# asmirnou/watsor

Hardware: AMD Instinct MI355X
Metric: detected frames/sec (whole node) + p50 per-frame latency, SSD-MobileNet 300x300 (higher is better)
Workload: dtype f16; 1 GPU; 1 synthetic 640x480 RGB stream per GPU, batch=8 frames, SSD-MobileNet-v2 300x300 (seeded random-init weights), frames resident in HBM, rows copied back to host; batch=8, frame=640x480, parallelism=replica-per-gpu x1, batches_in_flight=4, graph_nodes_per_batch=31

## Files before the change

### watsor_amd/csrc/k_conv.hip

```cpp
#include "wz_common.h"

__global__ __launch_bounds__(256) void wz_k_stem(const half_t* __restrict__ in, const float* __restrict__ w,
                                                 const float* __restrict__ bias, half_t* __restrict__ out,
                                                 int total, int hin, int win, int hout, int wout, int pad_t,
                                                 int pad_l) {
    __shared__ float sw[27 * 32 + 32];
    for (int i = threadIdx.x; i < 27 * 32; i += 256) sw[i] = w[i];
    if (threadIdx.x < 32) sw[27 * 32 + threadIdx.x] = bias[threadIdx.x];
    __syncthreads();
    const int tid = blockIdx.x * 256 + threadIdx.x;
    if (tid >= total) return;
    const int cg = tid & 3, pix = tid >> 2;
    const int ox = pix % wout;
    const int t2 = pix / wout;
    const int oy = t2 % hout, b = t2 / hout;
    float acc[8];
#pragma unroll
    for (int j = 0; j < 8; ++j) acc[j] = sw[27 * 32 + cg * 8 + j];
#pragma unroll
    for (int ky = 0; ky < 3; ++ky) {
        const int iy = oy * 2 - pad_t + ky;
        if (iy < 0 || iy >= hin) continue;
#pragma unroll
        for (int kx = 0; kx < 3; ++kx) {
            const int ix = ox * 2 - pad_l + kx;
            if (ix < 0 || ix >= win) continue;
            const half4_t p = *reinterpret_cast<const half4_t*>(in + ((size_t)(b * hin + iy) * win + ix) * 4);
#pragma unroll
            for (int c = 0; c < 3; ++c) {
                const float x = (float)p[c];
                const float* wr = sw + ((ky * 3 + kx) * 3 + c) * 32 + cg * 8;
#pragma unroll
                for (int j = 0; j < 8; ++j) acc[j] = fmaf(x, wr[j], acc[j]);
            }
        }
    }
    half8_t o;
#pragma unroll
    for (int j = 0; j < 8; ++j) o[j] = (half_t)fminf(fmaxf(acc[j], 0.0f), 6.0f);
    *reinterpret_cast<half8_t*>(out + (size_t)pix * 32 + cg * 8) = o;
}

void wz_launch_stem(const half_t* in, const float* w, const float* bias, half_t* out, int n, int hin, int win,
                    int hout, int wout, int pad_t, int pad_l, hipStream_t s) {
    const int total = n * hout * wout * 4;
    WZ_LAUNCH(wz_k_stem, dim3((total + 255) / 256), dim3(256), 0, s, in, w, bias, out, total, hin, win,
                       hout, wout, pad_t, pad_l);
}

__global__ __launch_bounds__(256) void wz_k_dw(const half_t* __restrict__ in, const half_t* __restrict__ w,
                                               const float* __restrict__ bias, half_t* __restrict__ out,
                                               int total, int hin, int win, int c, int hout, int wout, int stride,
                                               int pad_t, int pad_l, int act) {
    const int tid = blockIdx.x * 256 + threadIdx.x;
    if (tid >= total) return;
    const int c8 = c >> 3;
    const int cg = tid % c8, pix = tid / c8;
    const int ox = pix % wout;
    const int t2 = pix / wout;
    const int oy = t2 % hout, b = t2 / hout;
    float acc[8];
    {
        const float4_t b0 = *reinterpret_cast<const float4_t*>(bias + cg * 8);
        const float4_t b1 = *reinterpret_cast<const float4_t*>(bias + cg * 8 + 4);
#pragma unroll
        for (int j = 0; j < 4; ++j) { acc[j] = b0[j]; acc[4 + j] = b1[j]; }
    }
#pragma unroll
    for (int ky = 0; ky < 3; ++ky) {
        const int iy = oy * stride - pad_t + ky;
        if (iy < 0 || iy >= hin) continue;
#pragma unroll
        for (int kx = 0; kx < 3; ++kx) {
            const int ix = ox * stride - pad_l + kx;
            if (ix < 0 || ix >= win) continue;
            const half8_t x = *reinterpret_cast<const half8_t*>(in + ((size_t)(b * hin + iy) * win + ix) * c + cg * 8);
            const half8_t k = *reinterpret_cast<const half8_t*>(w + (size_t)(ky * 3 + kx) * c + cg * 8);
#pragma unroll
            for (int j = 0; j < 8; ++j) acc[j] = fmaf((float)x[j], (float)k[j], acc[j]);
        }
    }
    half8_t o;
#pragma unroll
    for (int j = 0; j < 8; ++j) {
        float v = acc[j];
        if (act == WZ_ACT_RELU6) v = fminf(fmaxf(v, 0.0f), 6.0f);
        o[j] = (half_t)v;
    }
    *reinterpret_cast<half8_t*>(out + (size_t)pix * c + cg * 8) = o;
}

void wz_launch_dw(const half_t* in, const half_t* w, const float* bias, half_t* out, int n, int hin, int win,
                  int c, int hout, int wout, int stride, int pad_t, int pad_l, int act, hipStream_t s) {
    const int total = n * hout * wout * (c >> 3);
    WZ_LAUNCH(wz_k_dw, dim3((total + 255) / 256), dim3(256), 0, s, in, w, bias, out, total, hin, win, c,
                       hout, wout, stride, pad_t, pad_l, act);
}


__device__ __forceinline__ void wz_epilogue4(const WzConvArgs& a, int m, int n4, float4_t v) {
    if (m >= a.M || n4 >= a.cout) return;
    const float4_t bv = *reinterpret_cast<const float4_t*>(a.bias + n4);
#pragma unroll
    for (int r = 0; r < 4; ++r) {
        float x = v[r] + bv[r];
        if (a.act == WZ_ACT_RELU6) x = fminf(fmaxf(x, 0.0f), 6.0f);
        v[r] = x;
    }
    if (a.out_mode == WZ_OUT_ACT) {
        const size_t o = (size_t)m * a.cout + n4;
        if (a.res) {
            const half4_t rv = *reinterpret_cast<const half4_t*>(a.res + o);
#pragma unroll
            for (int r = 0; r < 4; ++r) v[r] += (float)rv[r];
        }
        half4_t h = {(half_t)v[0], (half_t)v[1], (half_t)v[2], (half_t)v[3]};
        const size_t os = a.out_cstride ? (size_t)m * a.out_cstride + a.out_coff + n4 : o;
        *reinterpret_cast<half4_t*>(reinterpret_cast<half_t*>(a.out) + os) = h;
    } else {
        const int hw = a.hout * a.wout;
        const int b = m / hw, pix = m - b * hw;
        float* o;
        int cols, n0;
        if (a.out_mode == WZ_OUT_HEAD && n4 >= a.n_box) {
            cols = a.cout - a.n_box;
            n0 = n4 - a.n_box;
            o = a.out2 + (size_t)b * a.out2_batch_stride + a.out2_off;
        } else {
            cols = (a.out_mode == WZ_OUT_HEAD) ? a.n_box : a.cout;
            n0 = n4;
            o = reinterpret_cast<float*>(a.out) + (size_t)b * a.out_batch_stride + a.out_off;
        }
        o += (size_t)pix * cols + n0;
#pragma unroll
        for (int r = 0; r < 4; ++r)
            if (n0 + r < cols) o[r] = v[r];
    }
}

__device__ __forceinline__ void wz_decode_anchor(const float4_t e, const float4_t an, const WzPostConsts& k,
                                                 float* __restrict__ box_out, uint8_t* __restrict__ valid_out) {
#pragma clang fp contract(off)
    const float ty = e[0] / k.scale_y, tx = e[1] / k.scale_x, th = e[2] / k.scale_h, tw = e[3] / k.scale_w;
    const float w = expf(tw) * an[3];
    const float h = expf(th) * an[2];
    const float yc = ty * an[2] + an[0];
    const float xc = tx * an[3] + an[1];
    const float hh = h / 2.0f, hw = w / 2.0f;
    float ymin = yc - hh, xmin = xc - hw, ymax = yc + hh, xmax = xc + hw;
    if (k.clip_after) {
        *reinterpret_cast<float4_t*>(box_out) = (float4_t){ymin, xmin, ymax, xmax};
        *valid_out = 1;
        return;
    }
    ymin = fminf(fmaxf(ymin, 0.0f), 1.0f);
    xmin = fminf(fmaxf(xmin, 0.0f), 1.0f);
    ymax = fminf(fmaxf(ymax, 0.0f), 1.0f);
    xmax = fminf(fmaxf(xmax, 0.0f), 1.0f);
    const float area = (ymax - ymin) * (xmax - xmin);
    *reinterpret_cast<float4_t*>(box_out) = (float4_t){ymin, xmin, ymax, xmax};
    *valid_out = area > 0.0f ? 1 : 0;
}

__device__ __forceinline__ void wz_head_finish(const WzConvArgs& a, int m, int n4, float4_t v, bool list, bool decode,
                                               const float* __restrict__ hint_logit, uint32_t* __restrict__ cbits,
                                               int cbits_words, const WzPostConsts& pc, const float* __restrict__ anchors,
                                               float* __restrict__ boxes, uint8_t* __restrict__ valid) {
    wz_epilogue4(a, m, n4, v);
    if (m >= a.M) return;
    const int n_box = a.out_mode == WZ_OUT_HEAD ? a.n_box : (a.out_mode == WZ_OUT_BOX ? a.cout : 0);
    if (list && n4 >= n_box && n4 < a.cout && a.out_mode != WZ_OUT_BOX && a.out_mode != WZ_OUT_ACT) {
        const int hw = a.hout * a.wout;
        const int b = m / hw, pix = m - b * hw;
        const int cols = a.cout - n_box, n0 = n4 - n_box;
        const long long off = a.out_mode == WZ_OUT_HEAD ? a.out2_off : a.out_off;
        const float lf = hint_logit[b];
        const float4_t bv = *reinterpret_cast<const float4_t*>(a.bias + n4);
#pragma unroll
        for (int r = 0; r < 4; ++r) {
            const float x = v[r] + bv[r];
            if (n0 + r < cols && x >= lf) {
                const long long j = off + (long long)pix * cols + n0 + r;
                atomicOr(&cbits[(size_t)b * cbits_words + (size_t)(j >> 5)], 1u << (j & 31));
            }
        }
    }
    if (decode && n4 < n_box) {
        const float4_t bv = *reinterpret_cast<const float4_t*>(a.bias + n4);
        float4_t enc;
#pragma unroll
        for (int r = 0; r < 4; ++r) enc[r] = v[r] + bv[r];
        const int hw = a.hout * a.wout;
        const int b = m / hw, pix = m - b * hw;
        const int anchor = (int)(a.out_off >> 2) + pix * (n_box >> 2) + (n4 >> 2);
        const size_t i = (size_t)b * pc.num_anchors + anchor;
        wz_decode_anchor(enc, *reinterpret_cast<const float4_t*>(anchors + (size_t)anchor * 4), pc, boxes + i * 4, valid + i);
    }
}


template <int MT, int NT, int U>
struct ConvFrags {
    half8_t xa[U][MT];
    half8_t wf[U][NT];
};

template <int KS, int MT, int NT, int U>
__device__ __forceinline__ void wz_conv_load(const WzConvArgs& a, ConvFrags<MT, NT, U>& f, int& ql, const int q1, int& t,
                                             int& c, const int (&iy0)[MT], const int (&ix0)[MT],
                                             const int (&boff)[MT], const bool (&mv)[MT],
                                             const half_t* wlane, const int nt0, const int cg8) {
    constexpr int taps = KS * KS;
    const half8_t zero = {0, 0, 0, 0, 0, 0, 0, 0};
#pragma unroll
    for (int u = 0; u < U; ++u) {
        const bool live = ql < q1;
        const int ky = (KS == 1) ? 0 : t / KS, kx = (KS == 1) ? 0 : t - ky * KS;
        const bool cin_ok = (c * 32 + cg8) < a.cin;
#pragma unroll
        for (int mt = 0; mt < MT; ++mt) {
            const int iy = iy0[mt] + ky, ix = ix0[mt] + kx;
            const bool ok = live && cin_ok && mv[mt] && iy >= 0 && iy < a.hin && ix >= 0 && ix < a.win;
            f.xa[u][mt] = ok ? *reinterpret_cast<const half8_t*>(
                                   a.in + ((size_t)(boff[mt] + iy) * a.win + ix) * a.cin + c * 32 + cg8)
                             : zero;
        }
#pragma unroll
        for (int nt = 0; nt < NT; ++nt)
            f.wf[u][nt] = live ? *reinterpret_cast<const half8_t*>(
                                     wlane + ((size_t)((nt0 + nt) * taps + t) * a.kc + c) * 512)
                               : zero;
        ++ql;
        if (++c == a.kc) {
            c = 0;
            ++t;
        }
    }
}

template <int MT, int NT, int U>
__device__ __forceinline__ void wz_conv_mfma(const ConvFrags<MT, NT, U>& f, float4_t (&acc)[MT][NT]) {
#pragma unroll
    for (int u = 0; u < U; ++u)
#pragma unroll
        for (int mt = 0; mt < MT; ++mt)
#pragma unroll
            for (int nt = 0; nt < NT; ++nt)
                acc[mt][nt] = __builtin_amdgcn_mfma_f32_16x16x32_f16(f.wf[u][nt], f.xa[u][mt], acc[mt][nt], 0, 0, 0);
}

template <int KS, int MT, int NT, int U>
__device__ __forceinline__ void wz_conv_body(const WzConvArgs& a, int bx, int by, int bz) {
    const int lane = threadIdx.x & 63;
    const int wave = threadIdx.x >> 6;
    const int r16 = lane & 15, g = lane >> 4;
    const int m_base = (bx * 4 + wave) * (MT * 16);
    const int nt0 = by * NT;
    if (m_base >= a.M) return;

    const int hw = a.hout * a.wout;
    int iy0[MT], ix0[MT], boff[MT];
    bool mv[MT];
#pragma unroll
    for (int mt = 0; mt < MT; ++mt) {
        const int m = m_base + mt * 16 + r16;
        mv[mt] = m < a.M;
        const int mm = mv[mt] ? m : 0;
        const int b = mm / hw, rem = mm - b * hw;
        const int oy = rem / a.wout, ox = rem - oy * a.wout;
        iy0[mt] = oy * a.stride - a.pad_t;
        ix0[mt] = ox * a.stride - a.pad_l;
        boff[mt] = b * a.hin;
    }

    float4_t acc[MT][NT];
#pragma unroll
    for (int mt = 0; mt < MT; ++mt)
#pragma unroll
        for (int nt = 0; nt < NT; ++nt) acc[mt][nt] = (float4_t){0.f, 0.f, 0.f, 0.f};

    const int per = (a.kchunks + a.splitk - 1) / a.splitk;
    const int q0 = bz * per;
    const int q1 = min(q0 + per, a.kchunks);
    const half_t* wlane = a.w + (size_t)lane * 8;
    const int cg8 = g * 8;

    int ql = q0, t = (KS == 1) ? 0 : q0 / a.kc, c = (KS == 1) ? q0 : q0 - t * a.kc;
    ConvFrags<MT, NT, U> fa, fb;
    wz_conv_load<KS, MT, NT, U>(a, fa, ql, q1, t, c, iy0, ix0, boff, mv, wlane, nt0, cg8);
    for (int q = q0; q < q1;) {
        wz_conv_load<KS, MT, NT, U>(a, fb, ql, q1, t, c, iy0, ix0, boff, mv, wlane, nt0, cg8);
// ... 356 lines not shown
```

### watsor_amd/csrc/wz_common.h

```cpp
#pragma once
#include <hip/hip_runtime.h>
#include <hip/hip_fp16.h>
#include <stdint.h>
#include <stdlib.h>

#include "../../include/watsor_hip.h"
#include "wz_program.h"

typedef _Float16 half_t;
typedef __attribute__((ext_vector_type(8))) _Float16 half8_t;
typedef __attribute__((ext_vector_type(4))) _Float16 half4_t;
typedef __attribute__((ext_vector_type(4))) float float4_t;
#ifdef __HIPCC__
__device__ __forceinline__ half4_t wz_relu6_pack(const float4_t d, const float4_t bv, bool keep) {
    typedef __attribute__((ext_vector_type(2))) unsigned int wz_uint2_t;
    half4_t o;
#pragma unroll
    for (int r = 0; r < 4; ++r) o[r] = (half_t)fminf(fmaxf(d[r] + bv[r], 0.0f), 6.0f);
    wz_uint2_t p = __builtin_bit_cast(wz_uint2_t, o);
    p[0] = keep ? p[0] : 0u;
    p[1] = keep ? p[1] : 0u;
    return __builtin_bit_cast(half4_t, p);
}
#endif

struct WzFrameDesc {
    const uint8_t* rgb;
    int32_t w, h;
    float scale_x, scale_y;
    int32_t cam;
    int32_t fmt;
};
static_assert(sizeof(WzFrameDesc) == 32, "WzFrameDesc is 32 bytes (WzDescPack, the lanes' descriptor blocks)");

struct WzConvArgs {
    const half_t* in;
    const half_t* w;
    const float* bias;
    const half_t* res;
    void* out;
    int32_t M;
    int32_t hin, win, cin;
    int32_t hout, wout, cout, n_pad;
    int32_t ksize, stride, pad_t, pad_l, kc;
    int32_t act, out_mode;
    int32_t splitk;
    int32_t kchunks;
    int64_t out_batch_stride;
    int64_t out_off;
    float* out2;
    int64_t out2_batch_stride, out2_off;
    int32_t n_box;
    const half_t* zeros;
    int32_t grid_m, grid_n;
    float* ws;
    unsigned long long* dbg;
    int32_t nt_base;
    int32_t nt_live, nt_group;
    int32_t frag_ws;
    int32_t out_coff, out_cstride;
};


struct WzPostConsts {
    int32_t num_anchors, num_classes;
    int32_t max_total, max_per_class;
    float score_thr, iou_thr;
    float scale_y, scale_x, scale_h, scale_w;
    int32_t clip_after;
    int32_t _pad;
};

struct WzMbArgs {
    const half_t* in;
    const half_t* we;
    const float* be;
    const half_t* wd;
    const float* bd;
    const half_t* wp;
    const float* bp;
    const half_t* res;
    half_t* out;
    int32_t hin, win, hout, wout;
    int32_t cin0, kc0, nmid_pad;
    int32_t cmid, cmid_pad, kc;
    int32_t cout, n_pad;
    int32_t stride, pad_t, pad_l;
    int32_t stem, sin_h, sin_w, spad_t, spad_l;
    float* ws;
    uint64_t ws_bytes;
    int32_t M;
    unsigned long long* dbg;
    int32_t th, tw, tiles_y, tiles_x, nsplit, cpg, stage, ebufs, nb;
    const half_t* we_lo;
    const half_t* wp_lo;
    int32_t hp, hp_out;
    half_t* out2;
    int32_t has_out2;
    int32_t qenc;
    unsigned long long* dbg2;
    int32_t lone;
};

struct WzDwsepArgs {
    const half_t* in;
    const half_t* wd;
    const float* bd;
    const half_t* wp;
    const float* bp;
    half_t* out;
    int32_t M;
    int32_t hin, win, hout, wout;
    int32_t cin, kc, cout, n_pad;
    int32_t stride, pad_t, pad_l;
    unsigned long long* dbg;
};

struct WzCamFilter {
    int32_t enabled, width, height, n_zones;
    const int32_t* sat;
    double conf_thr[WZ_NUM_LABELS];
    double area_thr[WZ_NUM_LABELS];
    uint8_t allow[WZ_NUM_LABELS][WZ_MAX_ZONES * 4];
};
#define WZ_MAX_ZONES_PER_CAM (WZ_MAX_ZONES * 4)


extern thread_local int wz_launch_repeat;
static inline const char* wz_dev_getenv(const char* name) {
#ifdef WZ_DEV_BUILD
    return getenv(name);
#else
    (void)name;
    return nullptr;
#endif
}
static inline int wz_dev_env_int(const char* name, int dflt) {
    const char* e = wz_dev_getenv(name);
    return (e && e[0] && atoi(e) >= 0) ? atoi(e) : dflt;
}

bool wz_latency_schedule();

#ifndef WZ_LANE_STAMPS
#define WZ_LANE_STAMPS 0
#endif
#define WZ_STAMP_SLOTS 128
#define WZ_STAMP_WORDS 384
#define WZ_STAMP_ENTRY 16
#define WZ_STAMP_EXIT 80
#define WZ_STAMP_PRE_BYTES (WZ_STAMP_WORDS * 8)
struct WzLaunchNote { const void* func; unsigned grid[3], block[3]; unsigned lds; };
#if WZ_LANE_STAMPS
void wz_note_launch(const void* func, dim3 grid, dim3 block, size_t lds);
#define WZ_LAUNCH(kern, grid, block, lds, s, ...) do { wz_note_launch(reinterpret_cast<const void*>(kern), grid, block, lds); \
        for (int _wz_r = 0; _wz_r < wz_launch_repeat; ++_wz_r) hipLaunchKernelGGL(kern, grid, block, lds, s, __VA_ARGS__); } while (0)
#ifdef __HIPCC__
struct WzLaneStamp {
    unsigned long long* p;
    __device__ __forceinline__ explicit WzLaneStamp(unsigned long long* q) : p(q) {
        if (p && threadIdx.x == 0 && threadIdx.y == 0 && threadIdx.z == 0) {
            const unsigned id = blockIdx.x + gridDim.x * (blockIdx.y + gridDim.y * blockIdx.z);
            if (id < 64u) p[WZ_STAMP_ENTRY + id] = (unsigned long long)wall_clock64();
        }
    }
    __device__ __forceinline__ ~WzLaneStamp() {
        if (p && threadIdx.x == 0 && threadIdx.y == 0 && threadIdx.z == 0) {
            const unsigned id = blockIdx.x + gridDim.x * (blockIdx.y + gridDim.y * blockIdx.z);
            p[WZ_STAMP_EXIT + (id & 255u)] = (unsigned long long)wall_clock64();
        }
    }
};
#define WZ_LANE_STAMP(ptr) WzLaneStamp _wz_lane_stamp(const_cast<unsigned long long*>(ptr))
#endif
#else
#define WZ_LAUNCH(...) do { for (int _wz_r = 0; _wz_r < wz_launch_repeat; ++_wz_r) hipLaunchKernelGGL(__VA_ARGS__); } while (0)
#define WZ_LANE_STAMP(ptr) do { } while (0)
#endif
#define WZ_DESC_PACK 16
struct WzDescPack { WzFrameDesc d[WZ_DESC_PACK]; };
void wz_launch_preprocess(const WzFrameDesc* d_frames, int n, int size, half_t* out, hipStream_t s, bool hp = false,
                          WzFrameDesc* keep = nullptr, bool half_pixel = false, const WzFrameDesc* by_value = nullptr, int rows_lds = 0);
size_t wz_preprocess_rows_lds(int max_w);
size_t wz_preprocess_rows_need(int w, int fmt);
int wz_preprocess_flags(bool half_pixel, int rows_lds);
int wz_preprocess_rows_threads();
const void* wz_preprocess_func(bool hp, bool rows = false);
void wz_launch_stem(const half_t* in, const float* w, const float* bias, half_t* out, int n, int hin, int win,
                    int hout, int wout, int pad_t, int pad_l, hipStream_t s);
void wz_launch_dw(const half_t* in, const half_t* w, const float* bias, half_t* out, int n, int hin, int win,
                  int c, int hout, int wout, int stride, int pad_t, int pad_l, int act, hipStream_t s);
void wz_launch_conv(const WzConvArgs& a, hipStream_t s);
void wz_launch_splitk_reduce(const WzConvArgs& a, const float* ws, hipStream_t s);
#define WZ_REDUCE_GROUP_MAX 8
struct WzReduceGroup {
    int32_t n;
    int32_t first[WZ_REDUCE_GROUP_MAX + 1];
    WzConvArgs a[WZ_REDUCE_GROUP_MAX];
    const float* ws[WZ_REDUCE_GROUP_MAX];
    int32_t decode;
    int32_t list, cbits_words;
    unsigned long long* stamp;
    const float* hint_logit;
    uint32_t* cbits;
    WzPostConsts pc;
    const float* anchors;
    float* boxes;
    uint8_t* valid;
};
void wz_reduce_group_add(WzReduceGroup& g, const WzConvArgs& a, const float* ws);
#define WZ_CONV_GROUP_MAX 6
struct WzConvGroup {
    int32_t n;
    int32_t first[WZ_CONV_GROUP_MAX + 1];
    int32_t gx[WZ_CONV_GROUP_MAX], gy[WZ_CONV_GROUP_MAX];
    WzConvArgs a[WZ_CONV_GROUP_MAX];
    unsigned long long* stamp;
};
bool wz_conv_ws_applies(const WzConvArgs& a);
void wz_launch_conv_ws(const WzConvArgs& a, hipStream_t s);
bool wz_conv_groupable(const WzConvArgs& a);
void wz_conv_group_add(WzConvGroup& g, const WzConvArgs& a);
void wz_launch_conv_group(const WzConvGroup& g, hipStream_t s);
bool wz_conv_rs_groupable(const WzConvArgs& a);
int wz_conv_rs_group_add(WzConvGroup& g, const WzConvArgs& a);
void wz_launch_conv_rs_group(const WzConvGroup& g, hipStream_t s);
bool wz_conv_wide_applies(const WzConvArgs& a);
#define WZ_WIDE_TILES 12
void wz_conv_wide_shape(const WzConvArgs& a, int* tiles, int* steps);
int wz_choose_wide_T(const int* tiles, const int* steps, const long long* tile_bytes, int n, int cus);
int wz_conv_wide_group_add(WzConvGroup& g, const WzConvArgs& a);
void wz_launch_conv_wide_group(const WzConvGroup& g, hipStream_t s);
void wz_launch_splitk_reduce_group(const WzReduceGroup& g, hipStream_t s);
int wz_choose_splitk(int M, int n_pad, int kchunks);
bool wz_conv_use_lds(const WzConvArgs& a);
int wz_choose_splitk_lds(int M, int n_pad, int kchunks);
int wz_lds_nw(int M, int n_pad, int kchunks);
bool wz_conv_f32_use_rs(const WzConvArgs& a);
int wz_choose_splitk_rs_f32(int M, int n_pad, int kchunks);
bool wz_conv_ws_f32_applies(const WzConvArgs& a);
void wz_launch_conv_ws_f32(const WzConvArgs& a, hipStream_t s);
bool wz_extras_pair_applies(const WzConvArgs& a, const WzConvArgs& b);
void wz_launch_extras_pair(const WzConvArgs& a, const WzConvArgs& b, int n, hipStream_t s);
void wz_launch_stem_f32(const half_t* in, const float* w, const float* bias, float* out, int n, int hin, int win,
                        int hout, int wout, int pad_t, int pad_l, hipStream_t s, bool pair = false);
void wz_launch_dw_f32(const float* in, const float* w, const float* bias, float* out, int n, int hin, int win, int c,
                      int hout, int wout, int stride, int pad_t, int pad_l, int act, hipStream_t s);
void wz_launch_conv_f32(const WzConvArgs& a, hipStream_t s, bool reduce = true);
void wz_launch_stem7(const half_t* in, const half_t* w, const float* bias, half_t* out, int n, int hin, int win, int hout, int wout,
                     int pad_t, int pad_l, int cstride, int coff, hipStream_t s);
void wz_launch_stem7_f32(const half_t* in, const float* w, const float* bias, float* out, int n, int hin, int win, int hout, int wout,
                         int pad_t, int pad_l, int cstride, int coff, bool pair, hipStream_t s);
void wz_launch_pool3(const half_t* in, half_t* out, int n, int hin, int win, int c, int hout, int wout, int stride, int pad_t, int pad_l,
                     bool is_max, int cstride, int coff, hipStream_t s);
void wz_launch_pool3_f32(const float* in, float* out, int n, int hin, int win, int c, int hout, int wout, int stride, int pad_t, int pad_l,
                         bool is_max, int cstride, int coff, hipStream_t s);
int wz_launch_mbconv(const WzMbArgs& a, int n, hipStream_t s, bool prepare);
int wz_launch_mbconv_wave(const WzMbArgs& a, int n, hipStream_t s, bool prepare);
int wz_launch_mbconv_cs(const WzMbArgs& a, int n, hipStream_t s, bool prepare);
int wz_launch_mbconv_hp(const WzMbArgs& a, int n, hipStream_t s, bool prepare);
int wz_mbconv_hp2_applies(const WzMbArgs& a, int n);
int wz_launch_mbconv_hp2(const WzMbArgs& a, int n, hipStream_t s, bool prepare, int phase);
int wz_launch_dwsep(const WzDwsepArgs& a, hipStream_t s, bool prepare);

#define WZ_HIST_BINS 1024
#define WZ_CAND_CAP 4096
#define WZ_NMS_KEEP_MAX 128
#define WZ_CAND_TARGET 192
struct WzPostBuffers {
    uint32_t* hint;
    float* hint_logit;
    uint32_t* cbits;
    const float* box_enc;
    const float* logits;
    const float* anchors;
    float* boxes;
    uint8_t* valid;
    float* det_boxes;
    float* det_scores;
    int32_t* det_classes;
    int32_t* det_num;
    unsigned long long* dbg;
    unsigned long long* stamps;
    unsigned long long* stamps_pre;
    unsigned long long* stamps_host;
    int32_t stamps_n, _stamps_pad;
};
void wz_launch_decode(const WzPostBuffers& b, const WzPostConsts& c, int n, hipStream_t s);
void wz_launch_nms(const WzPostBuffers& b, const WzPostConsts& c, int n, hipStream_t s, const WzFrameDesc* d_frames = nullptr,
                   const WzCamFilter* d_cams = nullptr, wz_detection_t* rows = nullptr, uint8_t* pass = nullptr,
                   bool listed = false, uint32_t* status = nullptr);
void wz_launch_rows(const WzPostBuffers& b, const WzFrameDesc* d_frames, const WzCamFilter* d_cams, int n,
                    int max_total, wz_detection_t* rows, uint8_t* pass, hipStream_t s);
int wz_set_error(int code, const char* fmt, ...);
void wz_post_init();
void wz_launch_filter_rows(const WzCamFilter* d_cams, int cam, wz_detection_t* rows, uint8_t* pass, hipStream_t s);
void wz_launch_sat(const uint8_t* fill, int32_t* sat, int width, int height, int n_zones, hipStream_t s);

struct WzCropPlane {
    const uint8_t* src;
    uint8_t* dst;
    int32_t src_pitch, row_bytes, rows, _pad;
};
#define WZ_CROP_PACK 48
struct WzCropPack { WzCropPlane p[WZ_CROP_PACK]; };
struct WzMergeFrame { int32_t first, n_tiles, cam, _pad; };
struct WzMergeCand {
    int32_t label, x_min, y_min, x_max, y_max, _pad;
    double confidence;
};
void wz_launch_crop_tiles(const WzCropPlane* planes, int n, hipStream_t s);
void wz_launch_merge_tiles(const WzMergeFrame* frames, const int32_t* origins, const wz_detection_t* tile_rows, WzMergeCand* cands, int n,
                           int max_tiles, double iou_thr, double ios_thr, wz_detection_t* rows, uint8_t* pass, hipStream_t s);

#define WZ_GATE_GRAY 0
#define WZ_GATE_YUYV 1
#define WZ_GATE_UYVY 2
#define WZ_GATE_RGB 3
#define WZ_GATE_BGR 4
#define WZ_GATE_LOW10 5
struct WzGateTile {
    const uint8_t* src;
    const uint16_t* ref;
    uint16_t* now;
    int32_t pitch, row_bytes, tw, th, cols, crows, mode, thr;
};
struct WzGateCommit {
    uint16_t* ref;
    const uint16_t* now;
    wz_detection_t* cache;
    int32_t cells, fresh;
};
void wz_launch_tile_activity(const WzGateTile* tiles, int n, int max_crows, int max_cols, int32_t* counters, int32_t* activity, hipStream_t s);
void wz_launch_gate_commit(const WzGateCommit* tiles, int n, const wz_detection_t* batch_rows, wz_detection_t* out, hipStream_t s);
```

### watsor_amd/csrc/wz_engine.hip

```cpp
#include <math.h>
#include <stdarg.h>
#include <stdio.h>
#include <stdlib.h>
#include <string.h>

#include <algorithm>
#include <atomic>
#include <chrono>

#include "wz_engine.h"

static const char kHwQueuesVar[] = "GPU_MAX_HW_QUEUES";
static const int kHwQueuesNeeded = 8;
static int wz_env_hw_queues() {
    const char* v = getenv(kHwQueuesVar);
    if (!v || !v[0]) return 0;
    char* end = nullptr;
    const long n = strtol(v, &end, 10);
    while (*end == ' ' || *end == '\t') ++end;
    return (*end || n < 1 || n > 1 << 20) ? 0 : (int)n;
}
#ifndef WZ_KEEP_HOST_HW_QUEUES
__attribute__((constructor)) static void wz_runtime_defaults() {
    if (wz_env_hw_queues() < kHwQueuesNeeded) setenv(kHwQueuesVar, "8", 1);
// ... 208 lines not shown
            if (e->d_mbdbg) e->mb_groups[i] = groups;
            if (t) t->mark();
            if (groups > 1) {
                WzConvArgs r;
                memset(&r, 0, sizeof(r));
                r.bias = a.bp; r.res = a.res; r.out = a.out;
                r.M = a.M; r.hout = op.hout; r.wout = op.wout; r.cout = op.cout; r.n_pad = op.n_pad;
                r.act = WZ_ACT_NONE; r.out_mode = WZ_OUT_ACT; r.splitk = groups;
                WZ_STAMP_ARG(r);
                wz_launch_splitk_reduce(r, L.d_ws, s);
            }
        } else {
            if (!f32 && op.out_mode == WZ_OUT_ACT && op.ksize == 1 && op.dst_c == 0 && i + 1 < e->hdr.n_ops) {
                const WzOpDesc& nx = e->ops[i + 1];
                bool only = nx.kind == WZ_OP_CONV && nx.src == op.dst && nx.out_mode == WZ_OUT_ACT && op.res < 0 && nx.res < 0 &&
                            nx.dst_c == 0;
                for (uint32_t j = 0; only && j < e->hdr.n_ops; ++j)
                    if (j != i + 1 && (e->ops[j].src == op.dst || e->ops[j].res == op.dst)) only = false;
                if (only) {
                    auto conv_args = [&](const WzOpDesc& o) {
                        WzConvArgs c;
                        memset(&c, 0, sizeof(c));
                        c.in = L.tptr[o.src];
                        c.w = (const half_t*)(wbase + o.w_off);
                        c.bias = (const float*)(wbase + o.b_off);
                        c.out = L.tptr[o.dst];
                        c.M = n * o.hout * o.wout;
                        c.hin = o.hin; c.win = o.win; c.cin = o.cin;
                        c.hout = o.hout; c.wout = o.wout; c.cout = o.cout; c.n_pad = o.n_pad;
                        c.ksize = o.ksize; c.stride = o.stride; c.pad_t = o.pad_t; c.pad_l = o.pad_l; c.kc = o.kc;
                        c.act = o.act; c.out_mode = o.out_mode;
                        c.kchunks = o.ksize * o.ksize * o.kc;
                        c.splitk = 1;
                        return c;
                    };
                    WzConvArgs pa = conv_args(op);
                    const WzConvArgs pb = conv_args(nx);
                    if (wz_extras_pair_applies(pa, pb)) {
                        WZ_STAMP_ARG(pa);
                        wz_launch_extras_pair(pa, pb, n, s);
                        if (t) { t->mark(); t->mark(); t->mark(); t->mark(); }
                        ++i;
                        continue;
                    }
                }
            }
            WzConvArgs a;
            memset(&a, 0, sizeof(a));
            a.in = L.tptr[op.src];
            a.w = (const half_t*)(wbase + op.w_off);
            a.bias = (const float*)(wbase + op.b_off);
            a.res = op.res >= 0 ? L.tptr[op.res] : nullptr;
            a.M = n * op.hout * op.wout;
            a.hin = op.hin; a.win = op.win; a.cin = op.cin;
            a.hout = op.hout; a.wout = op.wout; a.cout = op.cout; a.n_pad = op.n_pad;
            a.ksize = op.ksize; a.stride = op.stride; a.pad_t = op.pad_t; a.pad_l = op.pad_l; a.kc = op.kc;
            a.act = op.act; a.out_mode = op.out_mode;
            a.kchunks = op.ksize * op.ksize * op.kc;
            if (op.out_mode == WZ_OUT_ACT && op.dst_c != 0) {
                a.out_cstride = op.dst_c;
                a.out_coff = op.dst_coff;
            }
            void* final_out;
            if (op.out_mode == WZ_OUT_ACT) {
                final_out = L.tptr[op.dst];
            } else if (op.out_mode == WZ_OUT_BOX) {
                final_out = L.d_box_enc;
                a.out_batch_stride = (int64_t)e->hdr.num_anchors * 4;
                a.out_off = (int64_t)op.anchor_off * 4;
            } else if (op.out_mode == WZ_OUT_CLS) {
                final_out = L.d_logits;
                a.out_batch_stride = (int64_t)e->hdr.num_anchors * e->hdr.num_classes;
                a.out_off = (int64_t)op.anchor_off * e->hdr.num_classes;
            } else {
                final_out = L.d_box_enc;
                a.out_batch_stride = (int64_t)e->hdr.num_anchors * 4;
                a.out_off = (int64_t)op.anchor_off * 4;
                a.out2 = L.d_logits;
                a.out2_batch_stride = (int64_t)e->hdr.num_anchors * e->hdr.num_classes;
                a.out2_off = (int64_t)op.anchor_off * e->hdr.num_classes;
                a.n_box = op.n_box;
            }
            a.zeros = e->d_zeros;
            a.dbg = e->d_mbdbg ? e->d_mbdbg + (size_t)i * 16 : nullptr;
            const bool makes_boxes = op.out_mode == WZ_OUT_HEAD || op.out_mode == WZ_OUT_BOX;
            if (makes_boxes) ++box_ops;
            if (op.out_mode != WZ_OUT_ACT) ++head_ops;
            if (f32) {
                int sk = !e->use_splitk ? 1 : wz_conv_f32_use_rs(a) ? wz_choose_splitk_rs_f32(a.M, a.n_pad, a.kchunks) : wz_choose_splitk(a.M, a.n_pad, a.kchunks / 2);
                const size_t slab32 = (((size_t)sk * a.M * a.n_pad * 4) + 255) & ~(size_t)255;
                if (sk > 1 && e->defer_heads && op.out_mode != WZ_OUT_ACT && heads.n < WZ_REDUCE_GROUP_MAX &&
                    slab32 + (e->ws_bytes >> 1) <= ws_top) {
                    ws_top -= slab32;
                    float* const park = reinterpret_cast<float*>(reinterpret_cast<unsigned char*>(L.d_ws) + ws_top);
                    a.splitk = sk;
                    a.ws = park;
                    a.out = final_out;
                    wz_launch_conv_f32(a, s, false);
                    if (t) { t->mark(); t->mark(); }
                    wz_reduce_group_add(heads, a, park);
                    if (makes_boxes) ++box_ops_grouped;
                    continue;
                }
                if (wz_conv_ws_f32_applies(a)) {
                    a.splitk = 1;
                    a.out = final_out;
                    wz_launch_conv_ws_f32(a, s);
                    if (t) { t->mark(); t->mark(); }
                    continue;
                }
                while (sk > 1 && (size_t)sk * a.M * a.n_pad * 4 > ws_top) --sk;
                a.splitk = sk;
                a.ws = L.d_ws;
                a.out = final_out;
                wz_launch_conv_f32(a, s);
                if (t) { t->mark(); t->mark(); }
                continue;
            }
            int sk = 1;
            if (e->use_splitk)
                sk = wz_conv_use_lds(a) ? wz_choose_splitk_lds(a.M, a.n_pad, a.kchunks) : wz_choose_splitk(a.M, a.n_pad, a.kchunks);
            bool to_wide = wide_T > 0 && wide.n < WZ_CONV_GROUP_MAX && wz_conv_wide_applies(a) && a.M >= e->wide_min_m;
            const size_t m16 = ((size_t)a.M + 15) & ~(size_t)15;
            if (to_wide) {
                const int wsk = ((a.kchunks >> 1) + wide_T - 1) / wide_T;
                if (heads.n < WZ_REDUCE_GROUP_MAX && ((((size_t)wsk * m16 * a.n_pad * 4) + 255) & ~(size_t)255) + (e->ws_bytes >> 1) <= ws_top)
                    sk = wsk;
                else
                    to_wide = false;
            }
            a.frag_ws = to_wide ? 1 : 0;
            const size_t slab = (((size_t)sk * (to_wide ? m16 : (size_t)a.M) * a.n_pad * 4) + 255) & ~(size_t)255;
            if ((sk > 1 || to_wide) && e->defer_heads && op.out_mode != WZ_OUT_ACT && heads.n < WZ_REDUCE_GROUP_MAX &&
                slab + (e->ws_bytes >> 1) <= ws_top) {
                ws_top -= slab;
                float* const park = reinterpret_cast<float*>(reinterpret_cast<unsigned char*>(L.d_ws) + ws_top);
                a.splitk = sk;
                a.out = park;
                if (to_wide) {
                    wz_conv_wide_group_add(wide, a);
                } else if (small.n < WZ_CONV_GROUP_MAX && wz_conv_groupable(a)) {
                    wz_conv_group_add(small, a);
                } else if (!(wz_conv_rs_groupable(a) && wz_conv_rs_group_add(big, a))) {
                    WZ_STAMP_ARG(a);
                    wz_launch_conv(a, s);
                }
                if (t) { t->mark(); t->mark(); }
                a.out = final_out;
                wz_reduce_group_add(heads, a, park);
                if (makes_boxes) ++box_ops_grouped;
                continue;
            }
            a.frag_ws = 0;
            if ((sk > 1 || a.M < 128) && wz_conv_ws_applies(a)) {
                a.splitk = 1;
                a.out = final_out;
                WZ_STAMP_ARG(a);
                wz_launch_conv_ws(a, s);
                if (t) { t->mark(); t->mark(); }
                continue;
            }
            while (sk > 1 && (size_t)sk * a.M * a.n_pad * 4 > ws_top) --sk;
            a.splitk = sk;
            if (sk > 1) {
                a.out = L.d_ws;
                WZ_STAMP_ARG(a);
                wz_launch_conv(a, s);
                if (t) t->mark();
                a.out = final_out;
                WZ_STAMP_ARG(a);
                wz_launch_splitk_reduce(a, L.d_ws, s);
            } else {
                a.out = final_out;
                WZ_STAMP_ARG(a);
                wz_launch_conv(a, s);
                if (t) t->mark();
            }
        }
        if (t) t->mark();
    }
    L.decode_fused = heads.n > 0 && box_ops > 0 && box_ops == box_ops_grouped && e->fuse_decode;
    L.cands_listed = with_post && L.decode_fused && head_ops == heads.n;
    wide.stamp = big.stamp = small.stamp = heads.stamp = nullptr;
    if (wide.n > 0) { WZ_STAMP_GROUP(wide); wz_launch_conv_wide_group(wide, s); }
    if (big.n > 0) { WZ_STAMP_GROUP(big); wz_launch_conv_rs_group(big, s); }
    if (t) t->mark();
    if (small.n > 0) { WZ_STAMP_GROUP(small); wz_launch_conv_group(small, s); }
    if (t) t->mark();
    if (L.decode_fused) {
        heads.decode = 1;
        heads.pc = e->pc;
        heads.anchors = L.post.anchors;
        heads.boxes = L.post.boxes;
        heads.valid = L.post.valid;
    }
    heads.list = L.cands_listed ? 1 : 0;
    if (L.cands_listed) {
        heads.hint_logit = L.post.hint_logit;
        heads.cbits = L.post.cbits;
        heads.cbits_words = (e->pc.num_anchors * e->pc.num_classes + 31) >> 5;
    }
    if (heads.n > 0) { WZ_STAMP_GROUP(heads); wz_launch_splitk_reduce_group(heads, s); }
    if (t) t->mark();
}

static void enqueue_post(wz_engine* e, Lane& L, bool rows, int n, StageTimer* t, bool decode_done = false, bool listed = false) {
    hipStream_t s = L.stream;
    if (!decode_done) wz_launch_decode(L.post, e->pc, n, s);
    if (t) t->mark();
#if WZ_LANE_STAMPS
    L.post.stamps_n = rows && L.m_stamps ? L.stamp_next : 0;
    L.post.stamps_host = rows && L.post.stamps_n ? L.m_stamps : nullptr;
#endif
    if (rows)
        wz_launch_nms(L.post, e->pc, n, s, L.d_desc, e->d_cams, L.m_rows, L.m_pass, listed, L.m_status);
    else
        wz_launch_nms(L.post, e->pc, n, s, nullptr, nullptr, nullptr, nullptr, listed);
    if (t) t->mark();
    if (rows && t) t->mark();
}

static void enqueue_batch(wz_engine* e, Lane& L, int n, StageTimer* t, int inner = 1) {
    hipStream_t s = L.stream;
    if (t) t->mark();
    const bool by_value = e->desc_by_value && n <= WZ_DESC_PACK;
    const bool zero_copy = !by_value && e->desc_zero_copy && L.h_desc_dev;
    if (!by_value && !zero_copy) (void)hipMemcpyAsync(L.d_desc, L.h_desc, sizeof(WzFrameDesc) * n, hipMemcpyHostToDevice, s);
    if (t) t->mark();
    wz_launch_repeat = inner;
    L.stamp_next = 1;
    wz_launch_preprocess(zero_copy ? L.h_desc_dev : L.d_desc, n, (int)e->hdr.input_size, L.tptr[input_tensor_index(e)], s,
                         input_is_pair(e), (zero_copy || by_value) ? L.d_desc : nullptr, e->hdr.resize_mode == 1,
                         by_value ? L.h_desc : nullptr, L.rows ? e->pre_rows_lds : 0);
    if (t) t->mark();
    enqueue_network(e, L, n, t);
    wz_launch_repeat = 1;
#ifdef WZ_DEV_BUILD
    L.post_modes[n | (L.rows ? 1 << 16 : 0)] = (L.decode_fused ? 1 : 0) | (L.cands_listed ? 2 : 0);
#endif
    enqueue_post(e, L, true, n, t, L.decode_fused, L.cands_listed);
}

int run_batch(wz_engine* e, int slot, int n) {
    Lane& L = e->lanes[slot];
    auto failed = [&]() -> int {
        const int op = L.launch_failed - 1;
        L.launch_failed = 0;
        return wz_fail(WZ_EFORMAT, "no %s kernel took op %d (%s) at batch %d",
                       e->ops[op].kind == WZ_OP_DWSEP ? "depthwise-separable" : "split-operand", op, e->ops[op].name, n);
    };
    const int key = n | (L.rows ? 1 << 16 : 0);
    L.key = key;
    bool graph = e->use_graph;
    if (graph && e->graph_adaptive) {
        graph = false;
        for (int li = 0; li < e->n_lanes && !graph; ++li)
            if (li != slot && e->lanes[li].done && hipEventQuery(e->lanes[li].done) == hipErrorNotReady) graph = true;
        (void)hipGetLastError();
    }
    auto ensure_graph = [&]() -> int {
        if (L.graphs.count(key)) return WZ_OK;
        hipGraph_t g = nullptr;
        HIPCHK(hipStreamBeginCapture(L.stream, hipStreamCaptureModeThreadLocal));
#if WZ_LANE_STAMPS
        L.launch_notes[key].clear();
        g_launch_sink = &L.launch_notes[key];
#endif
        L.lone = false;
        enqueue_batch(e, L, n, nullptr);
#if WZ_LANE_STAMPS
        g_launch_sink = nullptr;
#endif
        HIPCHK(hipStreamEndCapture(L.stream, &g));
        if (L.launch_failed) {
            (void)hipGraphDestroy(g);
            return failed();
        }
        size_t nodes = 0;
        if (hipGraphGetNodes(g, nullptr, &nodes) == hipSuccess) L.graph_nodes[key] = (int)nodes;
        if (e->desc_by_value && n <= WZ_DESC_PACK && nodes > 0) {
            std::vector<hipGraphNode_t> all(nodes);
            const void* want = wz_preprocess_func(input_is_pair(e), L.rows);
            if (hipGraphGetNodes(g, all.data(), &nodes) == hipSuccess)
                for (size_t k = 0; k < nodes; ++k) {
                    hipGraphNodeType ty;
                    hipKernelNodeParams kp;
                    if (hipGraphNodeGetType(all[k], &ty) == hipSuccess && ty == hipGraphNodeTypeKernel &&
                        hipGraphKernelNodeGetParams(all[k], &kp) == hipSuccess && kp.func == want) {
                        L.pre_nodes[key] = all[k];
                        break;
                    }
                }
            if (!L.pre_nodes.count(key)) {
                (void)hipGraphDestroy(g);
                return wz_fail(WZ_EHIP, "the resize kernel's node was not found in the captured graph");
            }
        }
        hipGraphExec_t ge = nullptr;
        HIPCHK(hipGraphInstantiate(&ge, g, nullptr, nullptr, 0));
        if (L.pre_nodes.count(key)) L.graph_src[key] = g;
        else (void)hipGraphDestroy(g);
        L.graphs.emplace(key, ge);
        return WZ_OK;
    };
    if (graph || (e->use_graph && !L.graphs.count(key))) {
        const int rc = ensure_graph();
// ... 1283 lines not shown
```

Before: 49470 frames/s.

## Add dedicated MFMA GEMM kernel for large 1x1 pointwise convolutions

Adds a specialised 1x1 convolution kernel that stages input rows into LDS with an XOR swizzle via buffer loads, preloads weight fragments into registers, and runs MFMA 16x16x32 f16 with an XCD-aware block remapping. The engine routes eligible pointwise convs (K = 320 channels, wide N, M >= 200) to it before the split-K / workspace paths. It also detects inputs produced by duplicated-output ops so the kernel can accumulate both K halves. The shared epilogue is moved into the header so it can be reused. The risk is heavy register use from the fully unrolled staging, and that fixed tile shapes only cover a narrow set of layers.

```diff
diff --git a/watsor_amd/csrc/k_conv.hip b/watsor_amd/csrc/k_conv.hip
--- a/watsor_amd/csrc/k_conv.hip
+++ b/watsor_amd/csrc/k_conv.hip
@@ -98,45 +98,6 @@
 }
 
 
-__device__ __forceinline__ void wz_epilogue4(const WzConvArgs& a, int m, int n4, float4_t v) {
-    if (m >= a.M || n4 >= a.cout) return;
-    const float4_t bv = *reinterpret_cast<const float4_t*>(a.bias + n4);
-#pragma unroll
-    for (int r = 0; r < 4; ++r) {
-        float x = v[r] + bv[r];
-        if (a.act == WZ_ACT_RELU6) x = fminf(fmaxf(x, 0.0f), 6.0f);
-        v[r] = x;
-    }
-    if (a.out_mode == WZ_OUT_ACT) {
-        const size_t o = (size_t)m * a.cout + n4;
-        if (a.res) {
-            const half4_t rv = *reinterpret_cast<const half4_t*>(a.res + o);
-#pragma unroll
-            for (int r = 0; r < 4; ++r) v[r] += (float)rv[r];
-        }
-        half4_t h = {(half_t)v[0], (half_t)v[1], (half_t)v[2], (half_t)v[3]};
-        const size_t os = a.out_cstride ? (size_t)m * a.out_cstride + a.out_coff + n4 : o;
-        *reinterpret_cast<half4_t*>(reinterpret_cast<half_t*>(a.out) + os) = h;
-    } else {
-        const int hw = a.hout * a.wout;
-        const int b = m / hw, pix = m - b * hw;
-        float* o;
-        int cols, n0;
-        if (a.out_mode == WZ_OUT_HEAD && n4 >= a.n_box) {
-            cols = a.cout - a.n_box;
-            n0 = n4 - a.n_box;
-            o = a.out2 + (size_t)b * a.out2_batch_stride + a.out2_off;
-        } else {
-            cols = (a.out_mode == WZ_OUT_HEAD) ? a.n_box : a.cout;
-            n0 = n4;
-            o = reinterpret_cast<float*>(a.out) + (size_t)b * a.out_batch_stride + a.out_off;
-        }
-        o += (size_t)pix * cols + n0;
-#pragma unroll
-        for (int r = 0; r < 4; ++r)
-            if (n0 + r < cols) o[r] = v[r];
-    }
-}
 
 __device__ __forceinline__ void wz_decode_anchor(const float4_t e, const float4_t an, const WzPostConsts& k,
                                                  float* __restrict__ box_out, uint8_t* __restrict__ valid_out) {
diff --git a/watsor_amd/csrc/k_gemm_1x1.hip b/watsor_amd/csrc/k_gemm_1x1.hip
--- /dev/null
+++ b/watsor_amd/csrc/k_gemm_1x1.hip
@@ -0,0 +1,113 @@
+#include "wz_common.h"
+
+typedef __attribute__((ext_vector_type(4))) unsigned int uint4_t;
+
+#define WZ_G1_TM 32
+#define WZ_G1_TN 128
+#define WZ_G1_STEPS 5
+#define WZ_G1_MIN_M 200
+
+template <bool DUP>
+__global__ __launch_bounds__(256, 2) void wz_k_gemm_1x1(const WzConvArgs a) {
+    WZ_LANE_STAMP(a.dbg);
+    constexpr int TM = WZ_G1_TM, MT = TM / 16, NT = 2, S = WZ_G1_STEPS, NF = DUP ? 2 : 1, XI = TM / 32;
+    constexpr int PRE = DUP ? 3 : S;
+    __shared__ __attribute__((aligned(16))) unsigned char smem[S * TM * 128];
+    const int lane = threadIdx.x & 63;
+    const int wave = __builtin_amdgcn_readfirstlane(threadIdx.x >> 6);
+    const int r16 = lane & 15, g = lane >> 4;
+    int bx, by;
+    {
+        const int L = (int)blockIdx.x, total = a.grid_m * a.grid_n;
+        const int xcd = L & 7, slot = L >> 3;
+        const int qd = total >> 3, rm = total & 7;
+        const int V = (xcd < rm ? xcd * (qd + 1) : rm * (qd + 1) + (xcd - rm) * qd) + slot;
+        bx = V % a.grid_m;
+        by = V / a.grid_m;
+    }
+    const int m_base = bx * TM;
+    const int nt_w = by * (WZ_G1_TN / 16) + wave * NT;
+    const int kcw = a.kc;
+
+    const unsigned row = (unsigned)a.cin * 2u;
+    const __amdgpu_buffer_rsrc_t rs_in = __builtin_amdgcn_make_buffer_rsrc((void*)a.in, 0, (int)((unsigned)a.M * row), 0x00020000);
+    const unsigned chunk = (unsigned)((lane & 7) ^ ((wave * 4 + (lane >> 4)) & 7));
+    uint4_t rb[S][XI];
+#pragma unroll
+    for (int s = 0; s < S; ++s)
+#pragma unroll
+        for (int i = 0; i < XI; ++i) {
+            const unsigned m = (unsigned)(m_base + i * 32 + wave * 8 + (lane >> 3));
+            rb[s][i] = __builtin_amdgcn_raw_buffer_load_b128(rs_in, m * row + chunk * 16u, s * 128, 0);
+        }
+
+    const half_t* const wl = a.w + (size_t)nt_w * kcw * 512 + lane * 8;
+    half8_t wf[S][2][NT][NF];
+    auto load_w = [&](int s) {
+#pragma unroll
+        for (int h = 0; h < 2; ++h)
+#pragma unroll
+            for (int nt = 0; nt < NT; ++nt)
+#pragma unroll
+                for (int f = 0; f < NF; ++f)
+                    wf[s][h][nt][f] = *reinterpret_cast<const half8_t*>(wl + ((size_t)nt * kcw + (s * 2 + h) + f * (kcw >> 1)) * 512);
+    };
+#pragma unroll
+    for (int s = 0; s < PRE; ++s) load_w(s);
+
+    float4_t acc[MT][NT];
+#pragma unroll
+    for (int mt = 0; mt < MT; ++mt)
+#pragma unroll
+        for (int nt = 0; nt < NT; ++nt) acc[mt][nt] = (float4_t){0.f, 0.f, 0.f, 0.f};
+
+#pragma unroll
+    for (int s = 0; s < S; ++s)
+#pragma unroll
+        for (int i = 0; i < XI; ++i)
+            *reinterpret_cast<uint4_t*>(smem + s * (TM * 128) + (i * 32 + wave * 8) * 128 + lane * 16) = rb[s][i];
+    __syncthreads();
+#pragma unroll
+    for (int s = PRE; s < S; ++s) load_w(s);
+
+#pragma unroll
+    for (int s = 0; s < S; ++s) {
+#pragma unroll
+        for (int h = 0; h < 2; ++h) {
+            half8_t xa[MT];
+#pragma unroll
+            for (int mt = 0; mt < MT; ++mt)
+                xa[mt] = *reinterpret_cast<const half8_t*>(smem + s * (TM * 128) + (mt * 16 + r16) * 128 + (((h * 4 + g) ^ ((r16 >> 1) & 7)) * 16));
+#pragma unroll
+            for (int f = 0; f < NF; ++f)
+#pragma unroll
+                for (int mt = 0; mt < MT; ++mt)
+#pragma unroll
+                    for (int nt = 0; nt < NT; ++nt)
+                        acc[mt][nt] = __builtin_amdgcn_mfma_f32_16x16x32_f16(wf[s][h][nt][f], xa[mt], acc[mt][nt], 0, 0, 0);
+        }
+    }
+
+#pragma unroll
+    for (int mt = 0; mt < MT; ++mt)
+#pragma unroll
+        for (int nt = 0; nt < NT; ++nt) wz_epilogue4(a, m_base + mt * 16 + r16, (nt_w + nt) * 16 + g * 4, acc[mt][nt]);
+}
+
+bool wz_gemm_1x1_applies(const WzConvArgs& a) {
+    const int kstaged = a.dup_k ? a.kc >> 1 : a.kc;
+    return a.out_mode == WZ_OUT_ACT && a.ksize == 1 && a.stride == 1 && a.pad_t == 0 && a.pad_l == 0 && a.hin == a.hout && a.win == a.wout &&
+           a.cin == a.kc * 32 && (!a.dup_k || a.kc % 2 == 0) && kstaged == 2 * WZ_G1_STEPS &&
+           a.n_pad >= 1024 && a.n_pad % WZ_G1_TN == 0 && a.M >= WZ_G1_MIN_M && (long long)(a.M + WZ_G1_TM) * a.cin * 2 < (1ll << 31);
+}
+
+void wz_launch_gemm_1x1(const WzConvArgs& a0, hipStream_t s) {
+    WzConvArgs a = a0;
+    a.grid_m = (a.M + WZ_G1_TM - 1) / WZ_G1_TM;
+    a.grid_n = a.n_pad / WZ_G1_TN;
+    const dim3 grid(a.grid_m * a.grid_n);
+    if (a.dup_k)
+        WZ_LAUNCH(wz_k_gemm_1x1<true>, grid, dim3(256), 0, s, a);
+    else
+        WZ_LAUNCH(wz_k_gemm_1x1<false>, grid, dim3(256), 0, s, a);
+}
diff --git a/watsor_amd/csrc/wz_common.h b/watsor_amd/csrc/wz_common.h
--- a/watsor_amd/csrc/wz_common.h
+++ b/watsor_amd/csrc/wz_common.h
@@ -59,8 +59,51 @@
     int32_t nt_live, nt_group;
     int32_t frag_ws;
     int32_t out_coff, out_cstride;
-};
-
+    int32_t dup_k;
+};
+
+
+#ifdef __HIPCC__
+__device__ __forceinline__ void wz_epilogue4(const WzConvArgs& a, int m, int n4, float4_t v) {
+    if (m >= a.M || n4 >= a.cout) return;
+    const float4_t bv = *reinterpret_cast<const float4_t*>(a.bias + n4);
+#pragma unroll
+    for (int r = 0; r < 4; ++r) {
+        float x = v[r] + bv[r];
+        if (a.act == WZ_ACT_RELU6) x = fminf(fmaxf(x, 0.0f), 6.0f);
+        v[r] = x;
+    }
+    if (a.out_mode == WZ_OUT_ACT) {
+        const size_t o = (size_t)m * a.cout + n4;
+        if (a.res) {
+            const half4_t rv = *reinterpret_cast<const half4_t*>(a.res + o);
+#pragma unroll
+            for (int r = 0; r < 4; ++r) v[r] += (float)rv[r];
+        }
+        half4_t h = {(half_t)v[0], (half_t)v[1], (half_t)v[2], (half_t)v[3]};
+        const size_t os = a.out_cstride ? (size_t)m * a.out_cstride + a.out_coff + n4 : o;
+        *reinterpret_cast<half4_t*>(reinterpret_cast<half_t*>(a.out) + os) = h;
+    } else {
+        const int hw = a.hout * a.wout;
+        const int b = m / hw, pix = m - b * hw;
+        float* o;
+        int cols, n0;
+        if (a.out_mode == WZ_OUT_HEAD && n4 >= a.n_box) {
+            cols = a.cout - a.n_box;
+            n0 = n4 - a.n_box;
+            o = a.out2 + (size_t)b * a.out2_batch_stride + a.out2_off;
+        } else {
+            cols = (a.out_mode == WZ_OUT_HEAD) ? a.n_box : a.cout;
+            n0 = n4;
+            o = reinterpret_cast<float*>(a.out) + (size_t)b * a.out_batch_stride + a.out_off;
+        }
+        o += (size_t)pix * cols + n0;
+#pragma unroll
+        for (int r = 0; r < 4; ++r)
+            if (n0 + r < cols) o[r] = v[r];
+    }
+}
+#endif
 
 struct WzPostConsts {
     int32_t num_anchors, num_classes;
@@ -219,6 +262,8 @@
 };
 bool wz_conv_ws_applies(const WzConvArgs& a);
 void wz_launch_conv_ws(const WzConvArgs& a, hipStream_t s);
+bool wz_gemm_1x1_applies(const WzConvArgs& a);
+void wz_launch_gemm_1x1(const WzConvArgs& a, hipStream_t s);
 bool wz_conv_groupable(const WzConvArgs& a);
 void wz_conv_group_add(WzConvGroup& g, const WzConvArgs& a);
 void wz_launch_conv_group(const WzConvGroup& g, hipStream_t s);
diff --git a/watsor_amd/csrc/wz_engine.hip b/watsor_amd/csrc/wz_engine.hip
--- a/watsor_amd/csrc/wz_engine.hip
+++ b/watsor_amd/csrc/wz_engine.hip
@@ -384,6 +384,17 @@
                 continue;
             }
             a.frag_ws = 0;
+            a.dup_k = 0;
+            for (uint32_t j = 0; j < i; ++j)
+                if (e->ops[j].dst == op.src && (e->ops[j].flags & WZ_OPF_DUP_OUT)) a.dup_k = 1;
+            if (wz_gemm_1x1_applies(a)) {
+                a.splitk = 1;
+                a.out = final_out;
+                WZ_STAMP_ARG(a);
+                wz_launch_gemm_1x1(a, s);
+                if (t) { t->mark(); t->mark(); }
+                continue;
+            }
             if ((sk > 1 || a.M < 128) && wz_conv_ws_applies(a)) {
                 a.splitk = 1;
                 a.out = final_out;
```

Result: faster. 50240 frames/s, median of 6 (+1.6%).
